# yzqin/s4g-release

Hardware: AMD Instinct MI355X
Metric: scenes/sec (25.6k-pt clouds) end-to-end grasp inference (higher is better)
Workload: dtype f32 (f16x2 split)

## Files before the change

### s4g_release_amd/csrc/mlp_gemm.hip

```cpp
#include <stdlib.h>

#include "mlp_common.h"

#include <type_traits>

#ifndef S4G_CHAIN_ABLATE
#define S4G_CHAIN_ABLATE 0
#endif

namespace s4g {


constexpr int GM_BM = 128;
constexpr int GM_BN = 128;
constexpr int GM_BK = 32;
constexpr int GM_LDS = 36;
constexpr int GM_THREADS = 256;

enum { LOAD_PLAIN = 0, LOAD_GATHER = 1, LOAD_INTERP = 2, LOAD_GATHER_MLP1 = 3, LOAD_GATHER_ADD = 4,
       LOAD_INTERP_ADD = 5, LOAD_CHANNEL_FIRST = 6,
       LOAD_REL_MLP1 = 64,
       LOAD_ADD_MFMA0 = 65 };
enum { EPI_STORE = 0, EPI_MAX = 1, EPI_CHANNEL_FIRST = 2, EPI_MAX_CF = 3 };

// ... 871 lines not shown
    for (int rb = 0; rb < 2; ++rb)
#pragma unroll
      for (int r = 0; r < 16; ++r) {
        const float v = acc[rb][cb][r] * sc;
        acc[rb][cb][r] = v;
        mx = fmaxf(mx, v);
        mn = fminf(mn, v);
      }
    const float hi = mx + bias, lo = mn + bias;
    tmax = fmaxf(tmax, p.relu ? hi : fmaxf(fabsf(hi), fabsf(lo)));
  }
  if (PL == 2 && po.out_amax) {
    const uint32_t wm = wave_max_u32(__float_as_uint(fmaxf(tmax, 0.f)));
    if (lane == 0) amax_publish(po.out_amax, wm, blockIdx.x * 4 + wave, p0, p_hi, p.rps);
  }
  if constexpr (EPI == EPI_MAX_CF)
    max_cf_epilogue<NCB>(po, acc, bg, p0, n0, wr, wc, li, lh, smemf);
  else
    gemm_epilogue<EPI, NCB>(po, acc, bg, g, p0, n0, wave, wr, wc, li, lh, smemf);
}

template <int LOADER, int EPI, int NCB, int PL>
static int launch_gemm_f16x2_cfg(GemmParams p, int groups, hipStream_t st) {
  constexpr int BN = 64 * NCB;
  p.ntiles = (p.Cout + BN - 1) / BN;
  size_t lds = sizeof(uint16_t) * PL * (GM_BM + BN) * GH_STR;
  const size_t epi = sizeof(float) * 4 * 32 * (32 * NCB + 4);
  if (lds < epi) lds = epi;
  static LdsAttrCache lds_cache;
  if (int rc = allow_dynamic_lds(reinterpret_cast<const void*>(&mlp_gemm_f16x2_kernel<LOADER, EPI, NCB, PL>), lds, lds_cache)) return rc;
  const dim3 grid((unsigned)(p.mtiles * p.ntiles), (unsigned)groups);
  hipLaunchKernelGGL((mlp_gemm_f16x2_kernel<LOADER, EPI, NCB, PL>), grid, dim3(256), lds, st, p);
  S4G_LAUNCH_CHECK();
  return S4G_OK;
}

__device__ __forceinline__ void chain_keep_alive(const f32x16& v) { asm volatile("" ::"v"(v)); }

#ifdef S4G_CHAIN_STAMPS
__device__ unsigned long long g_chain_stamps[512 * 16];
#define S4G_STAMP(i)                                                                       \
  do {                                                                                     \
    const unsigned sb_ = gridDim.x >= 1024 ? blockIdx.x - gridDim.x / 2 : blockIdx.x;    \
    if (threadIdx.x == 0 && sb_ < 512u && blockIdx.y == 0)                                 \
      g_chain_stamps[sb_ * 16 + (i)] = __builtin_amdgcn_s_memtime();                      \
  } while (0)
#else
#define S4G_STAMP(i)
#endif
constexpr int GF_RING_F16X2 = 2;
#ifndef S4G_CHAIN_RING1
#define S4G_CHAIN_RING1 2
#endif
#ifndef S4G_CHAIN_BF16_NRB
#define S4G_CHAIN_BF16_NRB 4
#endif

template <int LOADER, int EPI2, int RW, int KC, int PL>
__global__ __launch_bounds__(RW == 8 ? 512 : 256, (PL == 1 && RW != 8 && S4G_CHAIN_BF16_NRB == 2) ? 3 : 2) void mlp_chain_kernel(const GemmParams p) {
  constexpr int GF_RING = PL == 2 ? GF_RING_F16X2 : S4G_CHAIN_RING1;
  constexpr int NRB = PL == 1 ? S4G_CHAIN_BF16_NRB : 2, WROWS = 32 * NRB;
  constexpr int CW = RW == 8 ? 8 : 4 / RW, RWN = RW == 8 ? 1 : RW;
  constexpr int BM = WROWS * RWN, K = 64 * CW, NW = RWN * CW;
  constexpr int RS = 8 * NW, RPT = BM / RS;
  constexpr int astr = K + 8, aplane = BM * astr, KS = K >> 4;
  extern __shared__ __attribute__((aligned(16))) float smemf[];
  uint16_t* Ah = reinterpret_cast<uint16_t*>(smemf);
  float* scr = reinterpret_cast<float*>(Ah + PL * aplane);
  const int g = blockIdx.y;

  const int t = threadIdx.x;
  const int lane = t & 63;
  const int wave = t >> 6;

  constexpr bool ADD0 = LOADER == LOAD_ADD_MFMA0;
  constexpr bool ADD_BOUNDS = LOADER == LOAD_GATHER_ADD || LOADER == LOAD_INTERP_ADD || ADD0;
  constexpr bool MFMA0 = LOADER == LOAD_REL_MLP1;
  static_assert(!(MFMA0 || ADD0) || (PL == 2 && KC == 1), "phase 0 on the matrix cores: f16x2, one panel");
  static_assert(!ADD0 || EPI2 == EPI_MAX, "a wave's 64 rows are one centroid's neighbours");
  constexpr bool SEGMAX = (LOADER == LOAD_GATHER_MLP1 || MFMA0) && EPI2 == EPI_MAX;
  const int tile = blockIdx.x;
  const int p0 = tile * BM;
  bool seg_scene = false;
  if constexpr (SEGMAX) {
    if (p.seg_rows) {
      const int sc = p0 / p.rps;
      const int nrows = p.seg_rows[sc];
      if (p0 - sc * p.rps >= nrows) return;
      seg_scene = nrows < p.rps;
    }
  }
  const int p_hi = min(p0 + BM, p.P) - 1;
  const int am_s0 = p.rps > 0 ? p0 / p.rps : 0, am_s1 = p.rps > 0 ? p_hi / p.rps : 0;
  float am_v1 = 0.f, am_v2 = 0.f;
  if (PL == 2 && p.a_amax) am_v1 = p.a_amax[(size_t)am_s0 * 64 + lane];
  if (PL == 2 && p.a_amax2) am_v2 = p.a_amax2[(size_t)am_s0 * 64 + lane];

  const int wr = wave / CW, wc = wave % CW;
  const int li = lane & 31, lh = lane >> 5;
  const int wc_u = __builtin_amdgcn_readfirstlane(wc);
  const uint32_t wf_lane = (uint32_t)lane * 16u;
  constexpr size_t cb_stride = (size_t)KS * PL * 1024;
  constexpr size_t strip_stride = (size_t)CW * 2 * cb_stride;
  constexpr int kchunks = KC;
  const size_t cbs1 = (size_t)kchunks * cb_stride;
  const WRef w1 = wref(p.Wfrag + (size_t)g * p.Cout * p.Kpad16 * PL, (size_t)(wc_u * 2) * cbs1);
  const bool tri = p.Wfrag3 != nullptr;
  const WRef wmid = wref(p.Wfrag2 + (size_t)g * p.Cout2 * K * PL, (size_t)(wc_u * 2) * cb_stride);
  const int CoutF = tri ? p.Cout3 : p.Cout2;
  const float* __restrict__ scF = PL == 2 ? (tri ? p.w_inv_scale3 : p.w_inv_scale2) + (size_t)g * CoutF : nullptr;
  const float* __restrict__ bgF = (tri ? p.bias3 : p.bias2) + (size_t)g * CoutF;
  const WRef w2 = tri ? wref(p.Wfrag3 + (size_t)g * CoutF * K * PL, (size_t)(wc_u * 2) * cb_stride) : wmid;
  const int nstrip2 = (CoutF + 64 * CW - 1) / (64 * CW);
  const bool active0 = wc_u * 64 < CoutF;

  uint4 ring[GF_RING][2][PL];
#pragma unroll
  for (int d = 0; d < GF_RING; ++d)
#pragma unroll
    for (int cb = 0; cb < 2; ++cb)
#pragma unroll
      for (int pl = 0; pl < PL; ++pl)
        ring[d][cb][pl] = wref_load(w1, wf_lane + pl * 1024, (uint32_t)(cb * cbs1 + (size_t)d * PL * 1024));

  S4G_STAMP(0);
  ALoader<LOADER, RPT, RS> ld;
  float4 rv0[NRB];
  float4 wv0 = f4zero();
  constexpr int NKT0 = ADD0 ? K / 32 : 1, RPT0 = ADD0 ? RPT : 1;
  float4 fa[NKT0][RPT0];
  constexpr int fstr = K + 4;
  if constexpr (ADD0) {
    const int rows_left = p.P - p0;
    const __amdgpu_buffer_rsrc_t ridx = __builtin_amdgcn_make_buffer_rsrc(
        const_cast<int*>(p.gidx + p0), 0, (rows_left < BM ? rows_left : BM) * 4, 0x00020000);
    const __amdgpu_buffer_rsrc_t rxyz = __builtin_amdgcn_make_buffer_rsrc(
        const_cast<float*>(p.xyz), 0, p.nscenes * 3 * p.N * 4, 0x00020000);
    const __amdgpu_buffer_rsrc_t rfeat = __builtin_amdgcn_make_buffer_rsrc(
        const_cast<float*>(p.feat), 0, p.nscenes * p.N * p.Cf * 4, 0x00020000);
    constexpr uint32_t OOB = 0x80000000u;
    int jr[NRB], jg[RPT];
#pragma unroll
    for (int rb = 0; rb < NRB; ++rb)
      jr[rb] = __builtin_amdgcn_raw_buffer_load_b32(ridx, (wr * WROWS + rb * 32 + li) * 4, 0, 0);
#pragma unroll
    for (int s = 0; s < RPT; ++s) jg[s] = __builtin_amdgcn_raw_buffer_load_b32(ridx, ((t >> 3) + RS * s) * 4, 0, 0);
    {
      int bw, mw;
      gather_row_bm(p.M, p.K, p0, __builtin_amdgcn_readfirstlane(wr * WROWS), bw, mw);
      bw = __builtin_amdgcn_readfirstlane(bw);
      mw = __builtin_amdgcn_readfirstlane(mw);
      const bool okw = p0 + wr * WROWS < p.P;
      float cx = 0.f, cy = 0.f, cz = 0.f;
      if (okw) {
        const float* c = p.ctr + (size_t)bw * 3 * p.M + mw;
        cx = c[0];
        cy = c[p.M];
        cz = c[2 * p.M];
      }
      const uint32_t xb = okw ? (uint32_t)(bw * 3 * p.N) * 4u : OOB;
#pragma unroll
      for (int rb = 0; rb < NRB; ++rb) {
        const uint32_t vo = xb + (uint32_t)jr[rb] * 4u;
        const float x = __builtin_bit_cast(float, __builtin_amdgcn_raw_buffer_load_b32(rxyz, vo, 0, 0));
        const float y = __builtin_bit_cast(float, __builtin_amdgcn_raw_buffer_load_b32(rxyz, vo + (uint32_t)p.N * 4u, 0, 0));
        const float z = __builtin_bit_cast(float, __builtin_amdgcn_raw_buffer_load_b32(rxyz, vo + (uint32_t)p.N * 8u, 0, 0));
        rv0[rb] = make_float4(__fsub_rn(x, cx), __fsub_rn(y, cy), __fsub_rn(z, cz), 0.f);
      }
    }
    uint32_t rowoff[RPT];
#pragma unroll
    for (int s = 0; s < RPT; ++s) {
      const int c64 = (RS * s) / 64 * 64;
      int bc, mc;
      gather_row_bm(p.M, p.K, p0, c64, bc, mc);
      bc = __builtin_amdgcn_readfirstlane(bc);
      rowoff[s] = p0 + c64 < p.P ? (uint32_t)((bc * p.N + jg[s]) * p.Cf + (t & 7) * 4) * 4u : OOB;
    }
    if (p.Cin >= K) {
#pragma unroll
      for (int kt = 0; kt < NKT0; ++kt)
#pragma unroll
        for (int s = 0; s < RPT; ++s)
// ... 309 lines not shown
          tmax = fmaxf(fmaxf(tmax, fabsf(x[2])), fabsf(x[3]));
        }
      }
    }
  if constexpr (LOADER == LOAD_PLAIN && EPI2 == EPI_STORE) {
    if (!p.Wfrag2) {
      const bool second = p.split_n > 0 && g * p.c_gcol >= p.split_n;
      float* __restrict__ obase = second ? p.out2 - p.split_n : p.out + p.c_coff;
      const int old = second ? p.ldc2 : p.ldc;
      uint32_t* __restrict__ oamax = second ? p.out_amax2 : p.out_amax;
#pragma unroll
      for (int nb = 0; nb < 2; ++nb)
#pragma unroll
        for (int j = 0; j < 4; ++j) {
          const int nn = wc * 64 + nb * 32 + 8 * j + 4 * lh;
#pragma unroll
          for (int pb = 0; pb < NRB; ++pb) {
            const int row = p0 + wr * WROWS + pb * 32 + li;
            if (row < p.P)
              *reinterpret_cast<float4*>(obase + (size_t)row * old + g * p.c_gcol + nn) =
                  make_float4(acc[nb][pb][4 * j], acc[nb][pb][4 * j + 1], acc[nb][pb][4 * j + 2], acc[nb][pb][4 * j + 3]);
          }
        }
      if (PL == 2 && oamax) {
        const uint32_t wm = wave_max_u32(__float_as_uint(tmax));
        if (lane == 0) amax_publish(oamax, wm, (tile * 4 + wave) * 5 + g, p0, p_hi, p.rps);
      }
      return;
    }
  }
  float sh = 1.f;
  if constexpr (PL == 2) {
    const uint32_t wm = wave_max_u32(__float_as_uint(tmax));
    if (lane == 0) scr[NW * 128 + wave] = __uint_as_float(wm);
  }
  S4G_STAMP(5 + 4 * ph);
  __syncthreads();
  S4G_STAMP(6 + 4 * ph);
  if constexpr (PL == 2) {
    float hmax = scr[NW * 128];
#pragma unroll
    for (int w = 1; w < NW; ++w) hmax = fmaxf(hmax, scr[NW * 128 + w]);
    uint32_t exh = __float_as_uint(hmax) >> 23;
    exh = exh < 15u ? 15u : (exh > 240u ? 240u : exh);
    exh = __builtin_amdgcn_readfirstlane(exh);
    sh = __uint_as_float((268u - exh) << 23);
    inv_sh = __uint_as_float((exh - 14u) << 23);
  }
#pragma unroll
  for (int nb = 0; nb < 2; ++nb)
#pragma unroll
    for (int j = 0; j < 4; ++j)
#pragma unroll
      for (int pb = 0; pb < NRB; ++pb) {
        uint16_t* dst = Ah + (wr * WROWS + pb * 32 + li) * astr + wc * 64 + nb * 32 + 8 * j + 4 * lh;
        if constexpr (PL == 2) {
          const float4 v = make_float4(acc[nb][pb][4 * j], acc[nb][pb][4 * j + 1], acc[nb][pb][4 * j + 2],
                                       acc[nb][pb][4 * j + 3]);
          uint2 h, l;
          split2_h<false>(v, sh, h, l);
          *reinterpret_cast<uint2*>(dst) = h;
          *reinterpret_cast<uint2*>(dst + aplane) = l;
        } else {
          *reinterpret_cast<uint2*>(dst) = make_uint2(cvt_pk_bf16(acc[nb][pb][4 * j], acc[nb][pb][4 * j + 1]),
                                                      cvt_pk_bf16(acc[nb][pb][4 * j + 2], acc[nb][pb][4 * j + 3]));
        }
      }
  S4G_STAMP(7 + 4 * ph);
  __syncthreads();
  }
  inv_in = inv_sh;
  wcur = wmid;
  scp = PL == 2 ? p.w_inv_scale2 + (size_t)g * p.Cout2 : nullptr;
  bp = p.bias2 + (size_t)g * p.Cout2;
  relu_ph = p.relu2;
  }

  GemmParams q = p;
  q.Cout = CoutF;
  q.relu = tri ? p.relu3 : p.relu2;
  prime_a();
  WRef wstrip = w2;
  const float* __restrict__ bg2 = bgF;
  int sidv[NRB / 2][8] = {};
  if constexpr (SEGMAX) {
    if (seg_scene) {
#pragma unroll
      for (int c = 0; c < NRB / 2; ++c) {
        const int4* sp = reinterpret_cast<const int4*>(p.seg4 + ((p0 + wr * WROWS + c * 64 + lh * 32) >> 2));
        const int4 s0 = sp[0], s1 = sp[1];
        sidv[c][0] = s0.x; sidv[c][1] = s0.y; sidv[c][2] = s0.z; sidv[c][3] = s0.w;
        sidv[c][4] = s1.x; sidv[c][5] = s1.y; sidv[c][6] = s1.z; sidv[c][7] = s1.w;
      }
    }
  }
  for (int strip = 0; strip < nstrip2; ++strip, wstrip = wstrip + strip_stride) {
    if ((strip * CW + wc_u) * 64 >= CoutF) break;
    const int n = (strip * CW + wc) * 64 + lane;
    const float e_sc = PL == 2 ? inv_sh * scF[n] : 1.f;
    const float e_bias = bg2[n];
    const WRef wnext = ((strip + 1) * CW + wc_u) * 64 < CoutF ? wstrip + strip_stride : wstrip;
    S4G_STAMP(12 + 2 * (strip & 1));
    S4G_F2_STRIP(EPI2 == EPI_STORE, true, wstrip, cb_stride, wnext, cb_stride)
    S4G_STAMP(13 + 2 * (strip & 1));
    if (S4G_CHAIN_ABLATE & 8) {
      chain_keep_alive(acc[0][0]); chain_keep_alive(acc[0][1]); chain_keep_alive(acc[1][0]); chain_keep_alive(acc[1][1]);
      continue;
    }
    const int n0 = (strip * CW + wc) * 64;
    float omax = 0.f;
    if constexpr (EPI2 == EPI_STORE) {
      epi_s[lane] = e_sc;
      epi_s[64 + lane] = e_bias;
#pragma unroll
      for (int nb = 0; nb < 2; ++nb)
#pragma unroll
        for (int j = 0; j < 4; ++j) {
          const int nn = n0 + nb * 32 + 8 * j + 4 * lh;
          const float4 sc4 = *reinterpret_cast<const float4*>(epi_s + nb * 32 + 8 * j + 4 * lh);
          const float4 b4 = *reinterpret_cast<const float4*>(epi_s + 64 + nb * 32 + 8 * j + 4 * lh);
          const float scv[4] = {sc4.x, sc4.y, sc4.z, sc4.w};
          const float bv[4] = {b4.x, b4.y, b4.z, b4.w};
#pragma unroll
          for (int pb = 0; pb < NRB; ++pb) {
            float v[4];
#pragma unroll
            for (int e = 0; e < 4; ++e) {
              float x = __fmaf_rn(acc[nb][pb][4 * j + e], scv[e], bv[e]);
              if (q.relu) x = fmaxf(x, 0.f);
              v[e] = x;
              omax = fmaxf(omax, fabsf(x));
            }
            const int row = p0 + wr * WROWS + pb * 32 + li;
            if (row < p.P)
              *reinterpret_cast<float4*>(p.out + (size_t)row * p.ldc + p.c_coff + g * p.c_gcol + nn) =
                  make_float4(v[0], v[1], v[2], v[3]);
          }
        }
      if (p.out_amax) {
        const uint32_t wm = wave_max_u32(__float_as_uint(omax));
        if (lane == 0) amax_publish(p.out_amax, wm, tile * 4 + wave + strip, p0, p_hi, p.rps);
      }
    } else if (SEGMAX && seg_scene) {
      uint32_t* __restrict__ outu = reinterpret_cast<uint32_t*>(p.out);
#pragma unroll
      for (int cb = 0; cb < 2; ++cb) {
        const float sc = __shfl(e_sc, cb * 32 + li);
        const float bias = __shfl(e_bias, cb * 32 + li);
        const int nn = n0 + cb * 32 + li;
#pragma unroll
        for (int c = 0; c < NRB / 2; ++c) {
        float v[8];
#pragma unroll
        for (int qd = 0; qd < 4; ++qd) {
          const float o0 = fmaxf(fmaxf(acc[cb][2 * c][4 * qd], acc[cb][2 * c][4 * qd + 1]),
                                 fmaxf(acc[cb][2 * c][4 * qd + 2], acc[cb][2 * c][4 * qd + 3]));
          const float o1 = fmaxf(fmaxf(acc[cb][2 * c + 1][4 * qd], acc[cb][2 * c + 1][4 * qd + 1]),
                                 fmaxf(acc[cb][2 * c + 1][4 * qd + 2], acc[cb][2 * c + 1][4 * qd + 3]));
          const auto r = __builtin_amdgcn_permlane32_swap(__float_as_uint(o0), __float_as_uint(o1), false, false);
          v[2 * qd] = __uint_as_float(r[0]);
          v[2 * qd + 1] = __uint_as_float(r[1]);
        }
        auto emit = [&](int seg, float m) {
          if (seg < 0) return;
          const float x = fmaxf(m * sc + bias, 0.f);
          omax = fmaxf(omax, x);
          if (nn < CoutF) atomicMax(outu + (size_t)seg * p.ldc + p.c_coff + nn, __float_as_uint(x));
        };
        int cur = sidv[c][0];
        float m = v[0];
#pragma unroll
        for (int i = 1; i < 8; ++i) {
          const bool chg = sidv[c][i] != cur;
          if (chg) emit(cur, m);
          m = chg ? v[i] : fmaxf(m, v[i]);
          cur = sidv[c][i];
        }
        emit(cur, m);
        }
      }
      if (PL == 2 && p.out_amax) {
        const uint32_t wm = wave_max_u32(__float_as_uint(omax));
        if (lane == 0) amax_publish(p.out_amax, wm, tile * 4 + wave + strip, p0, p_hi, p.rps);
      }
    } else if (q.relu && p.K == 64) {
#pragma unroll
      for (int cb = 0; cb < 2; ++cb) {
        const float sc = __shfl(e_sc, cb * 32 + li);
        const float bias = __shfl(e_bias, cb * 32 + li);
        const int nn = n0 + cb * 32 + li;
#pragma unroll
        for (int c = 0; c < NRB / 2; ++c) {
          float m = acc[cb][2 * c][0];
#pragma unroll
          for (int rb = 2 * c; rb < 2 * c + 2; ++rb)
#pragma unroll
            for (int r = 0; r < 16; ++r) m = fmaxf(m, acc[cb][rb][r]);
          m = fmaxf(m, __shfl_xor(m, 32));
          const float v = fmaxf(m * sc + bias, 0.f);
          omax = fmaxf(omax, v);
          const int row0 = p0 + wr * WROWS + c * 64;
          if (nn < CoutF && lh == 0 && row0 < p.P) p.out[(size_t)(row0 >> 6) * p.ldc + p.c_coff + nn] = v;
        }
      }
      if (PL == 2 && p.out_amax) {
        const uint32_t wm = wave_max_u32(__float_as_uint(omax));
        if (lane == 0) amax_publish(p.out_amax, wm, tile * 4 + wave + strip, p0, p_hi, p.rps);
      }
    } else if constexpr (NRB == 2) {
      f32x16 acct[2][2];
#pragma unroll
      for (int cb = 0; cb < 2; ++cb) {
        const float sc = __shfl(e_sc, cb * 32 + li);
        const float bias = __shfl(e_bias, cb * 32 + li);
        float mx = -__builtin_inff(), mn = __builtin_inff();
#pragma unroll
        for (int rb = 0; rb < 2; ++rb)
#pragma unroll
          for (int r = 0; r < 16; ++r) {
            const float v = acc[cb][rb][r] * sc;
            acct[rb][cb][r] = v;
            mx = fmaxf(mx, v);
            mn = fminf(mn, v);
          }
        const float hi = mx + bias, lo = mn + bias;
        omax = fmaxf(omax, q.relu ? hi : fmaxf(fabsf(hi), fabsf(lo)));
      }
      if (p.out_amax) {
        const uint32_t wm = wave_max_u32(__float_as_uint(fmaxf(omax, 0.f)));
        if (lane == 0) amax_publish(p.out_amax, wm, tile * 4 + wave + strip, p0, p_hi, p.rps);
      }
      gemm_epilogue<EPI_MAX, 2>(q, acct, bg2, g, p0, n0, wave, wr, 0, li, lh, smemf);
    }
  }
  S4G_STAMP(11);
#undef S4G_F2_STRIP
#undef S4G_F2_TERM
}

template <int LOADER, int EPI2, int RW, int KC, int PL>
static int launch_mlp_chain(const GemmParams& p, int groups, hipStream_t st) {
  constexpr int CW = RW == 8 ? 8 : 4 / RW, RWN = RW == 8 ? 1 : RW;
  constexpr int NRB = PL == 1 ? S4G_CHAIN_BF16_NRB : 2;
  constexpr int BM = 32 * NRB * RWN, K = 64 * CW, NW = RWN * CW;
  constexpr size_t lds = sizeof(uint16_t) * PL * BM * (size_t)(K + 8) + sizeof(float) * (NW * 128 + 16);
  static_assert(lds <= (RW == 8 ? 160 : 80) * 1024, "two workgroups per CU (one for the 8-wave form)");
  static LdsAttrCache lds_cache;
  if (int rc = allow_dynamic_lds(reinterpret_cast<const void*>(&mlp_chain_kernel<LOADER, EPI2, RW, KC, PL>), lds, lds_cache)) return rc;
  const dim3 grid((unsigned)((p.P + BM - 1) / BM), (unsigned)groups);
  hipLaunchKernelGGL((mlp_chain_kernel<LOADER, EPI2, RW, KC, PL>), grid, dim3(64 * NW), lds, st, p);
  S4G_LAUNCH_CHECK();
  return S4G_OK;
}

template <int LOADER, int EPI, int PL = 2>
static int launch_gemm_f16x2(const GemmParams& p, int groups, hipStream_t st) {
  constexpr int force = 0;
  const int64_t wide_wgs = (int64_t)((p.P + GM_BM - 1) / GM_BM) * ((p.Cout + 255) / 256) * groups;
  const bool wide = force ? force == 4
                          : p.Cout > 256 && wide_wgs >= 512 &&
                                (LOADER == LOAD_PLAIN || LOADER == LOAD_GATHER_MLP1 || LOADER == LOAD_GATHER_ADD);
  if (wide) return launch_gemm_f16x2_cfg<LOADER, EPI, 4, PL>(p, groups, st);
  return launch_gemm_f16x2_cfg<LOADER, EPI, 2, PL>(p, groups, st);
}

template <int LOADER, int EPI, int NS, int WAVES>
static int launch_gemm_bf16x3_cfg(const GemmParams& p, int groups, hipStream_t st) {
  constexpr int BK = 32 * NS;
  size_t lds = sizeof(float) * GM_BM * (BK + 4) + sizeof(uint16_t) * 3 * GM_BN * (BK + 8);
  const size_t epi = sizeof(float) * 4 * 32 * 68;
  if (lds < epi) lds = epi;
  static LdsAttrCache lds_cache;
  if (int rc = allow_dynamic_lds(reinterpret_cast<const void*>(&mlp_gemm_bf16x3_kernel<LOADER, EPI, NS, WAVES>), lds, lds_cache)) return rc;
  const dim3 grid((unsigned)(p.mtiles * p.ntiles), (unsigned)groups);
  hipLaunchKernelGGL((mlp_gemm_bf16x3_kernel<LOADER, EPI, NS, WAVES>), grid, dim3(64 * WAVES), lds,
                     st, p);
  S4G_LAUNCH_CHECK();
  return S4G_OK;
}

template <int LOADER, int EPI>
static int launch_gemm_bf16x3(const GemmParams& p, int groups, hipStream_t st) {
  return launch_gemm_bf16x3_cfg<LOADER, EPI, 1, 4>(p, groups, st);
}

template <int LOADER, int EPI>
static int launch_gemm(const GemmParams& p, int groups, hipStream_t st) {
  const size_t lds = sizeof(float) * 2 * (GM_BM + GM_BN) * GM_LDS;
  static LdsAttrCache lds_cache;
  if (int rc = allow_dynamic_lds(reinterpret_cast<const void*>(&mlp_gemm_kernel<LOADER, EPI>), lds, lds_cache)) return rc;
  const dim3 grid((unsigned)(p.mtiles * p.ntiles), (unsigned)groups);
  hipLaunchKernelGGL((mlp_gemm_kernel<LOADER, EPI>), grid, dim3(GM_THREADS), lds, st, p);
  S4G_LAUNCH_CHECK();
  return S4G_OK;
}

}

#define S4G_FUSED2_LIST(X)                                                                       \
  X(LOAD_GATHER_MLP1, EPI_MAX, 2, 1)                                                             \
  X(LOAD_GATHER_MLP1, EPI_MAX, 1, 1)                                                             \
  X(LOAD_GATHER_ADD, EPI_MAX, 2, 1)                                                              \
  X(LOAD_GATHER_ADD, EPI_MAX, 1, 1)                                                              \
  X(LOAD_GATHER_ADD, EPI_MAX, 8, 1)       \
  X(LOAD_PLAIN, EPI_MAX, 2, 1)                                                                   \
  X(LOAD_PLAIN, EPI_MAX, 1, 1)                                                                   \
  X(LOAD_PLAIN, EPI_MAX, 8, 1)                                                                   \
  X(LOAD_PLAIN, EPI_STORE, 2, 1)                                                                 \
  X(LOAD_PLAIN, EPI_STORE, 1, 1)                                                                 \
  X(LOAD_PLAIN, EPI_STORE, 1, 2)            \
  X(LOAD_PLAIN, EPI_STORE, 1, 4)         \
  X(LOAD_PLAIN, EPI_STORE, 8, 1)                                                                 \
  X(LOAD_INTERP_ADD, EPI_STORE, 2, 1)                                                            \
  X(LOAD_INTERP_ADD, EPI_STORE, 1, 1)                                                            \
  X(LOAD_INTERP_ADD, EPI_STORE, 8, 1)

// ... 14 lines not shown
#undef S4G_FUSED2_Q
  return 0;
}

extern "C" int s4g_mlp_gemm_f32(const s4g_gemm_desc_t* d, s4g_stream_t stream) {
  using namespace s4g;
  if (!d || d->P < 0 || d->Cout <= 0 || d->groups <= 0 || !d->bias) return S4G_EINVAL;
  const bool split = d->precision == S4G_GEMM_BF16X3 || d->precision == S4G_GEMM_BF16;
  const bool h2 = d->precision == S4G_GEMM_F16X2;
  if (h2) {
    if (!d->W_f16x2 || !d->w_inv_scale || d->Kpad16 <= 0 || (d->Kpad16 & 15) ||
        !(d->a_amax_floor >= 0.f) || (!d->a_amax && !d->a_amax2 && !(d->a_amax_floor > 0.f)))
      return S4G_EINVAL;
  } else if (split) {
    if (!d->W_bf16x3 || d->Kpad16 <= 0 || (d->Kpad16 & 15)) return S4G_EINVAL;
  } else if (d->precision == S4G_GEMM_FP32) {
    if (!d->W || d->Kpad <= 0 || (d->Kpad & 7)) return S4G_EINVAL;
  } else {
    return S4G_EINVAL;
  }
  if (d->P == 0) return S4G_OK;
  GemmParams p;
  p.P = d->P; p.Cin = d->Cin; p.Kpad = d->Kpad; p.Cout = d->Cout; p.relu = d->relu;
  p.W = d->W; p.bias = d->bias;
  p.A = d->A; p.lda = d->lda; p.a_coff = d->a_coff; p.a_gcol = d->a_gcol; p.aL = d->a_L;
  p.gidx = d->gidx; p.feat = d->feat; p.xyz = d->xyz; p.ctr = d->ctr;
  p.Cf = d->Cf; p.N = d->N; p.M = d->M; p.K = d->K;
  p.nscenes = d->M > 0 && d->K > 0 ? (int)((d->P + (int64_t)d->M * d->K - 1) / ((int64_t)d->M * d->K)) : 0;
  p.mlp1 = (const float4*)d->mlp1_w;
  p.rel4 = (const float4*)d->rel_xyz4;
  p.seg4 = d->seg4;
  p.seg_rows = d->seg_rows;
  p.out2 = d->out2;
  p.ldc2 = d->ldc2;
  p.split_n = d->out2 ? d->split_n : 0;
  p.out_amax2 = (uint32_t*)d->out_amax2;
  p.nidx = d->nidx; p.nw = d->nw; p.sparse = d->sparse; p.dense = d->dense;
  p.C2 = d->C2; p.C1 = d->C1; p.N2 = d->N2; p.N1 = d->N1;
  p.out = d->out; p.ldc = d->ldc; p.c_coff = d->c_coff; p.c_gcol = d->c_gcol;
  p.w_gstride = d->w_gstride; p.b_gstride = d->b_gstride;
  for (int i = 0; i < 4; ++i) p.cf_ptr[i] = d->cf_ptr[i];
  for (int i = 0; i < 5; ++i) p.cf_start[i] = d->cf_start[i];
  p.cf_sigmoid_from = d->cf_sigmoid_from; p.cf_N = d->cf_N;
  p.W3 = (const uint16_t*)d->W_bf16x3;
  p.Kpad16 = d->Kpad16;
  p.bf16_single = d->precision == S4G_GEMM_BF16 ? 1 : 0;
  p.w3_plane = (size_t)d->groups * (size_t)d->Cout * (size_t)d->Kpad16;
  p.Wh2 = (const uint16_t*)d->W_f16x2;
  p.w_inv_scale = d->w_inv_scale;
  p.a_amax = d->a_amax; p.a_amax2 = d->a_amax2; p.a_amax_floor = d->a_amax_floor;
  p.out_amax = (uint32_t*)d->out_amax;
  p.rps = d->rows_per_scene > 0 ? d->rows_per_scene : 0;
  p.Wfrag = (const uint16_t*)d->W_f16x2_frag;
  p.lbias = d->loader_bias;
  p.Wfrag2 = (const uint16_t*)d->W2_f16x2_frag;
  p.w_inv_scale2 = d->w2_inv_scale;
  p.bias2 = d->bias2;
  p.Cout2 = d->Cout2;
  p.relu2 = d->relu2;
  p.Wfrag3 = (const uint16_t*)d->W3_f16x2_frag;
  p.w_inv_scale3 = d->w3_inv_scale;
  p.bias3 = d->bias3;
  p.Cout3 = d->Cout3;
  p.relu3 = d->relu3;
  p.mtiles = (d->P + GM_BM - 1) / GM_BM;
  p.ntiles = (d->Cout + GM_BN - 1) / GM_BN;
  hipStream_t st = (hipStream_t)stream;

  if (d->loader == S4G_GEMM_LOAD_PLAIN) {
    if (!d->A || (d->lda & 3) || (d->a_coff & 3) || (d->a_gcol & 3) || (d->Cin & 3)) return S4G_EINVAL;
  } else if (d->loader == S4G_GEMM_LOAD_GATHER) {
    if (!d->gidx || !d->xyz || !d->ctr || (d->Cf & 3) || (d->Cf > 0 && !d->feat) ||
        d->K <= 0 || d->M <= 0 || d->N <= 0 || d->groups != 1)
      return S4G_EINVAL;
  } else if (d->loader == S4G_GEMM_LOAD_GATHER_MLP1) {
    if ((!d->rel_xyz4 && (!d->gidx || !d->xyz || !d->ctr)) || ((uintptr_t)d->rel_xyz4 & 15) ||
        !d->mlp1_w || (d->Cin & 3) || d->K <= 0 || d->M <= 0 || d->N <= 0 || d->groups != 1 ||
        ((uintptr_t)d->mlp1_w & 15))
      return S4G_EINVAL;
    if ((d->seg4 != nullptr) != (d->seg_rows != nullptr)) return S4G_EINVAL;
    if (d->seg4 && (!d->rel_xyz4 || !d->W2_f16x2_frag || d->epilogue != S4G_GEMM_EPI_MAX || d->K != 64 ||
                    d->rows_per_scene <= 0 || (d->rows_per_scene & 255) || !d->relu2 || d->W3_f16x2_frag))
      return S4G_EINVAL;
  } else if (d->loader == S4G_GEMM_LOAD_GATHER_ADD) {
    if (!d->gidx || !d->xyz || !d->ctr || !d->mlp1_w || !d->feat || (d->Cin & 3) || d->Cf != d->Cin ||
        d->K <= 0 || d->M <= 0 || d->N <= 0 || d->groups != 1 || ((uintptr_t)d->mlp1_w & 15) ||
        ((uintptr_t)d->feat & 15))
      return S4G_EINVAL;
  } else if (d->loader == S4G_GEMM_LOAD_INTERP_ADD) {
    if (!d->nidx || !d->nw || !d->sparse || !d->loader_bias || (d->Cin & 3) || d->C2 != d->Cin ||
        d->N1 <= 0 || d->N2 <= 0 || d->groups != 1 ||
        (((uintptr_t)d->sparse | (uintptr_t)d->dense | (uintptr_t)d->loader_bias) & 15))
      return S4G_EINVAL;
  } else if (d->loader == S4G_GEMM_LOAD_INTERP) {
    if (!d->nidx || !d->nw || !d->sparse || (d->C2 & 3) || (d->C1 & 3) ||
        (d->C1 > 0 && !d->dense) || d->N1 <= 0 || d->N2 <= 0 || d->groups != 1)
      return S4G_EINVAL;
  } else if (d->loader == S4G_GEMM_LOAD_CHANNEL_FIRST) {
    if (!d->A || d->Cin < 1 || d->a_L <= 0 || d->P % d->a_L || d->groups != 1 ||
        d->Cin > (h2 ? d->Kpad16 : d->Kpad))
      return S4G_EINVAL;
  } else {
    return S4G_EINVAL;
  }
  if (d->loader != S4G_GEMM_LOAD_GATHER_MLP1 && (d->seg4 || d->seg_rows)) return S4G_EINVAL;
  if (d->out2) {
    const bool bf1_ = d->precision == S4G_GEMM_BF16;
    if (!(h2 || bf1_) || d->loader != S4G_GEMM_LOAD_PLAIN || d->epilogue != S4G_GEMM_EPI_STORE || d->W2_f16x2_frag ||
        d->groups != 1 || d->split_n <= 0 || (d->split_n & 255) || d->split_n >= d->Cout || (d->Cout & 255) ||
        (d->ldc2 & 3) || ((uintptr_t)d->out2 & 15) || d->c_coff != 0 || (d->ldc & 3) || ((uintptr_t)d->out & 15))
      return S4G_EINVAL;
  }
  if (d->epilogue == S4G_GEMM_EPI_MAX) {
    if (!(d->K == 16 || d->K == 32 || d->K == 64) || d->groups != 1 || !d->out) return S4G_EINVAL;
  } else if (d->epilogue == S4G_GEMM_EPI_STORE) {
    if (!d->out) return S4G_EINVAL;
  } else if (d->epilogue == S4G_GEMM_EPI_CHANNEL_FIRST) {
    if (d->cf_N <= 0 || d->groups != 1) return S4G_EINVAL;
  } else if (d->epilogue == S4G_GEMM_EPI_MAX_CHANNEL_FIRST) {
    if (d->relu != 1 || d->K < 1 || d->M < 1 || d->P % ((int64_t)d->M * d->K) || d->groups != 1 || !d->out ||
        d->W2_f16x2_frag || d->out2)
      return S4G_EINVAL;
  } else {
    return S4G_EINVAL;
  }

  if (d->W2_f16x2_frag) {
    const bool c128 = d->Cout == 128 && d->Kpad16 == 128,
               c256 = d->Cout == 256 && (d->Kpad16 == 256 || d->Kpad16 == 512 || d->Kpad16 == 1024),
               c512 = d->Cout == 512 && d->Kpad16 == 512;
    const bool store = d->epilogue == S4G_GEMM_EPI_STORE;
    const bool bf1 = d->precision == S4G_GEMM_BF16;
    if ((!h2 && !bf1) || (!store && (d->epilogue != S4G_GEMM_EPI_MAX || d->K != 64 || (d->P & 63))) ||
        (!c128 && !c256 && !c512) || d->Cout2 <= 0 || (d->Cout2 & 63) || (!store && d->groups != 1) || !d->W_f16x2_frag ||
        (d->W3_f16x2_frag && (d->Cout2 != d->Cout || d->Cout3 <= 0 || (d->Cout3 & 63) ||
                              (h2 && !d->w3_inv_scale) || !d->bias3)) ||
        (h2 && !d->w2_inv_scale) || !d->bias2 ||
        (store && (((d->ldc | d->c_coff | d->c_gcol) & 3) || ((uintptr_t)d->out & 15))))
      return S4G_EINVAL;
    if (bf1 && !store && !(d->W3_f16x2_frag ? d->relu3 : d->relu2)) return S4G_EUNSUPPORTED;
    if (h2 && d->loader == S4G_GEMM_LOAD_GATHER_MLP1 && d->rel_xyz4 && d->epilogue == S4G_GEMM_EPI_MAX &&
        d->Kpad16 == d->Cout && d->Cin <= d->Cout && (c128 || c256)) {
      const char* m0 = s4g::knob("S4G_MLP1_MFMA");
      if (!(m0 && m0[0] == '0'))
        return c128 ? launch_mlp_chain<LOAD_REL_MLP1, EPI_MAX, 2, 1, 2>(p, d->groups, st)
                    : launch_mlp_chain<LOAD_REL_MLP1, EPI_MAX, 1, 1, 2>(p, d->groups, st);
    }
    if (h2 && d->loader == S4G_GEMM_LOAD_GATHER_ADD && d->epilogue == S4G_GEMM_EPI_MAX && d->Kpad16 == d->Cout &&
        (int64_t)p.nscenes * d->N * d->Cf * 4 < (1ll << 31) && (int64_t)p.nscenes * d->N * 12 < (1ll << 31))
      return c128   ? launch_mlp_chain<LOAD_ADD_MFMA0, EPI_MAX, 2, 1, 2>(p, d->groups, st)
             : c256 ? launch_mlp_chain<LOAD_ADD_MFMA0, EPI_MAX, 1, 1, 2>(p, d->groups, st)
                    : launch_mlp_chain<LOAD_ADD_MFMA0, EPI_MAX, 8, 1, 2>(p, d->groups, st);
#define S4G_FUSED2_CASE(L, E, R, KCH)                                                        \
  if (d->loader == L && (int)d->epilogue == (int)E && (c128 ? 2 : (c256 ? 1 : 8)) == R &&     \
      d->Kpad16 / d->Cout == KCH)                                                             \
    return bf1 ? launch_mlp_chain<L, E, R, KCH, 1>(p, d->groups, st)                 \
               : launch_mlp_chain<L, E, R, KCH, 2>(p, d->groups, st);
    S4G_FUSED2_LIST(S4G_FUSED2_CASE)
#undef S4G_FUSED2_CASE
    return S4G_EUNSUPPORTED;
  }
  {
    const char* sc_env = s4g::knob("S4G_GEMM_SINGLE_CHAIN");
    const bool single_chain = !(sc_env && sc_env[0] == '0');
    const bool bf1 = d->precision == S4G_GEMM_BF16;
    const int kc = d->Kpad16 / 256;
// ... 74 lines not shown
```

Before: 1992.

## Streamline fused MLP chain max epilogues: precomputed segment offsets, single amax publish

Reworks the epilogue of the fused MLP chain kernel. Segment ids are loaded once per tile and redistributed by shuffle, with the atomic target byte offsets and segment-boundary limits precomputed outside the strip loop, so the segmented max needs fewer branches and less address arithmetic. The per-column scale and bias loads now avoid shuffles, the K=64 max path reduces halves with permlane32_swap and has all lanes store, and the amax reduction and publish happen once per wave after all strips instead of once per strip. In exchange, register pressure rises from the precomputed per-segment arrays, and a host check rejects outputs whose offsets would not fit in 32 bits.

```diff
diff --git a/s4g_release_amd/csrc/mlp_gemm.hip b/s4g_release_amd/csrc/mlp_gemm.hip
--- a/s4g_release_amd/csrc/mlp_gemm.hip
+++ b/s4g_release_amd/csrc/mlp_gemm.hip
@@ -977,12 +977,14 @@
   const int tile = blockIdx.x;
   const int p0 = tile * BM;
   bool seg_scene = false;
+  int seg_tile = -1;
   if constexpr (SEGMAX) {
     if (p.seg_rows) {
       const int sc = p0 / p.rps;
       const int nrows = p.seg_rows[sc];
       if (p0 - sc * p.rps >= nrows) return;
       seg_scene = nrows < p.rps;
+      if (lane < BM / 4) seg_tile = p.seg4[(p0 >> 2) + lane];
     }
   }
   const int p_hi = min(p0 + BM, p.P) - 1;
@@ -993,7 +995,7 @@
 
   const int wr = wave / CW, wc = wave % CW;
   const int li = lane & 31, lh = lane >> 5;
-  const int wc_u = __builtin_amdgcn_readfirstlane(wc);
+  const int wc_u = __builtin_amdgcn_readfirstlane(wc), wr_u = __builtin_amdgcn_readfirstlane(wr);
   const uint32_t wf_lane = (uint32_t)lane * 16u;
   constexpr size_t cb_stride = (size_t)KS * PL * 1024;
   constexpr size_t strip_stride = (size_t)CW * 2 * cb_stride;
@@ -1469,23 +1471,47 @@
   prime_a();
   WRef wstrip = w2;
   const float* __restrict__ bg2 = bgF;
-  int sidv[NRB / 2][8] = {};
+  constexpr uint32_t SEG_NONE = 0xFFFFFFFFu;
+  uint32_t seg_off[NRB / 2][8] = {};
+  float seg_lim[NRB / 2][8] = {};
+  uint32_t seg_any[NRB / 2] = {};
   if constexpr (SEGMAX) {
     if (seg_scene) {
 #pragma unroll
       for (int c = 0; c < NRB / 2; ++c) {
-        const int4* sp = reinterpret_cast<const int4*>(p.seg4 + ((p0 + wr * WROWS + c * 64 + lh * 32) >> 2));
-        const int4 s0 = sp[0], s1 = sp[1];
-        sidv[c][0] = s0.x; sidv[c][1] = s0.y; sidv[c][2] = s0.z; sidv[c][3] = s0.w;
-        sidv[c][4] = s1.x; sidv[c][5] = s1.y; sidv[c][6] = s1.z; sidv[c][7] = s1.w;
-      }
-    }
-  }
+        int sid[8];
+#pragma unroll
+        for (int i = 0; i < 8; ++i) sid[i] = __shfl(seg_tile, wr * (WROWS / 4) + c * 16 + lh * 8 + i);
+        uint32_t mine = 0u;
+#pragma unroll
+        for (int i = 0; i < 8; ++i) {
+          const bool ends = i == 7 || sid[i + 1] != sid[i];
+          const bool merges = ends && sid[i] >= 0;
+          seg_off[c][i] = merges ? ((uint32_t)sid[i] * (uint32_t)p.ldc + (uint32_t)p.c_coff + (uint32_t)li) * 4u : SEG_NONE;
+          seg_lim[c][i] = (i > 0 && sid[i] != sid[i - 1]) ? -__builtin_inff() : __builtin_inff();
+          mine |= merges ? 1u << i : 0u;
+        }
+        seg_any[c] = __builtin_amdgcn_readlane(mine, 0) | __builtin_amdgcn_readlane(mine, 32);
+      }
+    }
+  }
+  float omax = 0.f;
   for (int strip = 0; strip < nstrip2; ++strip, wstrip = wstrip + strip_stride) {
     if ((strip * CW + wc_u) * 64 >= CoutF) break;
-    const int n = (strip * CW + wc) * 64 + lane;
-    const float e_sc = PL == 2 ? inv_sh * scF[n] : 1.f;
-    const float e_bias = bg2[n];
+    const int n0u = (strip * CW + wc_u) * 64;
+    constexpr bool PER_BLOCK = EPI2 != EPI_STORE && SEGMAX;
+    [[maybe_unused]] float e_sc = 1.f, e_bias = 0.f, sc2[2] = {1.f, 1.f}, bias2[2] = {0.f, 0.f};
+    if constexpr (!PER_BLOCK) {
+      const int n = (PL == 2 ? n0u : (strip * CW + wc) * 64) + lane;
+      e_sc = PL == 2 ? inv_sh * scF[n] : 1.f;
+      e_bias = bg2[n];
+    } else {
+#pragma unroll
+      for (int cb = 0; cb < 2; ++cb) {
+        sc2[cb] = PL == 2 ? inv_sh * scF[n0u + cb * 32 + li] : 1.f;
+        bias2[cb] = bg2[n0u + cb * 32 + li];
+      }
+    }
     const WRef wnext = ((strip + 1) * CW + wc_u) * 64 < CoutF ? wstrip + strip_stride : wstrip;
     S4G_STAMP(12 + 2 * (strip & 1));
     S4G_F2_STRIP(EPI2 == EPI_STORE, true, wstrip, cb_stride, wnext, cb_stride)
@@ -1495,7 +1521,6 @@
       continue;
     }
     const int n0 = (strip * CW + wc) * 64;
-    float omax = 0.f;
     if constexpr (EPI2 == EPI_STORE) {
       epi_s[lane] = e_sc;
       epi_s[64 + lane] = e_bias;
@@ -1524,82 +1549,78 @@
                   make_float4(v[0], v[1], v[2], v[3]);
           }
         }
-      if (p.out_amax) {
-        const uint32_t wm = wave_max_u32(__float_as_uint(omax));
-        if (lane == 0) amax_publish(p.out_amax, wm, tile * 4 + wave + strip, p0, p_hi, p.rps);
-      }
     } else if (SEGMAX && seg_scene) {
-      uint32_t* __restrict__ outu = reinterpret_cast<uint32_t*>(p.out);
+      char* __restrict__ outb = reinterpret_cast<char*>(p.out + n0u);
 #pragma unroll
       for (int cb = 0; cb < 2; ++cb) {
-        const float sc = __shfl(e_sc, cb * 32 + li);
-        const float bias = __shfl(e_bias, cb * 32 + li);
-        const int nn = n0 + cb * 32 + li;
+        const float sc = sc2[cb], bias = bias2[cb];
+        const bool nn_ok = n0u + cb * 32 + li < CoutF;
 #pragma unroll
         for (int c = 0; c < NRB / 2; ++c) {
         float v[8];
 #pragma unroll
         for (int qd = 0; qd < 4; ++qd) {
-          const float o0 = fmaxf(fmaxf(acc[cb][2 * c][4 * qd], acc[cb][2 * c][4 * qd + 1]),
-                                 fmaxf(acc[cb][2 * c][4 * qd + 2], acc[cb][2 * c][4 * qd + 3]));
-          const float o1 = fmaxf(fmaxf(acc[cb][2 * c + 1][4 * qd], acc[cb][2 * c + 1][4 * qd + 1]),
-                                 fmaxf(acc[cb][2 * c + 1][4 * qd + 2], acc[cb][2 * c + 1][4 * qd + 3]));
+          const float o0 = fmaxf(fmaxf(fmaxf(acc[cb][2 * c][4 * qd], acc[cb][2 * c][4 * qd + 1]), acc[cb][2 * c][4 * qd + 2]),
+                                 acc[cb][2 * c][4 * qd + 3]);
+          const float o1 = fmaxf(fmaxf(fmaxf(acc[cb][2 * c + 1][4 * qd], acc[cb][2 * c + 1][4 * qd + 1]),
+                                       acc[cb][2 * c + 1][4 * qd + 2]), acc[cb][2 * c + 1][4 * qd + 3]);
           const auto r = __builtin_amdgcn_permlane32_swap(__float_as_uint(o0), __float_as_uint(o1), false, false);
           v[2 * qd] = __uint_as_float(r[0]);
           v[2 * qd + 1] = __uint_as_float(r[1]);
         }
-        auto emit = [&](int seg, float m) {
-          if (seg < 0) return;
-          const float x = fmaxf(m * sc + bias, 0.f);
-          omax = fmaxf(omax, x);
-          if (nn < CoutF) atomicMax(outu + (size_t)seg * p.ldc + p.c_coff + nn, __float_as_uint(x));
-        };
-        int cur = sidv[c][0];
         float m = v[0];
 #pragma unroll
-        for (int i = 1; i < 8; ++i) {
-          const bool chg = sidv[c][i] != cur;
-          if (chg) emit(cur, m);
-          m = chg ? v[i] : fmaxf(m, v[i]);
-          cur = sidv[c][i];
-        }
-        emit(cur, m);
-        }
-      }
-      if (PL == 2 && p.out_amax) {
-        const uint32_t wm = wave_max_u32(__float_as_uint(omax));
-        if (lane == 0) amax_publish(p.out_amax, wm, tile * 4 + wave + strip, p0, p_hi, p.rps);
+        for (int i = 0; i < 8; ++i) {
+          if (i > 0) m = fmaxf(fminf(m, seg_lim[c][i]), v[i]);
+          if (seg_any[c] & (1u << i)) {
+            if (seg_off[c][i] != SEG_NONE) {
+              const float x = fmaxf(m * sc + bias, 0.f);
+              omax = fmaxf(omax, x);
+              uint32_t off = seg_off[c][i];
+              asm volatile("" : "+v"(off));
+              if (nn_ok) atomicMax(reinterpret_cast<uint32_t*>(outb + cb * 128 + off), __float_as_uint(x));
+            }
+          }
+        }
+        }
       }
     } else if (q.relu && p.K == 64) {
-#pragma unroll
-      for (int cb = 0; cb < 2; ++cb) {
-        const float sc = __shfl(e_sc, cb * 32 + li);
-        const float bias = __shfl(e_bias, cb * 32 + li);
-        const int nn = n0 + cb * 32 + li;
-#pragma unroll
-        for (int c = 0; c < NRB / 2; ++c) {
-          float m = acc[cb][2 * c][0];
-#pragma unroll
-          for (int rb = 2 * c; rb < 2 * c + 2; ++rb)
-#pragma unroll
-            for (int r = 0; r < 16; ++r) m = fmaxf(m, acc[cb][rb][r]);
-          m = fmaxf(m, __shfl_xor(m, 32));
-          const float v = fmaxf(m * sc + bias, 0.f);
-          omax = fmaxf(omax, v);
+      const float sc = PER_BLOCK ? (lh ? sc2[1] : sc2[0]) : e_sc, bias = PER_BLOCK ? (lh ? bias2[1] : bias2[0]) : e_bias;
+      const int nn = n0 + lane;
+#pragma unroll
+      for (int c = 0; c < NRB / 2; ++c) {
+        float mb[2];
+#pragma unroll
+        for (int cb = 0; cb < 2; ++cb) {
+          float mr[2];
+#pragma unroll
+          for (int rb = 0; rb < 2; ++rb) {
+            float m = acc[cb][2 * c + rb][0];
+#pragma unroll
+            for (int r = 1; r < 15; r += 2) m = fmaxf(fmaxf(m, acc[cb][2 * c + rb][r]), acc[cb][2 * c + rb][r + 1]);
+            mr[rb] = m;
+          }
+          mb[cb] = fmaxf(fmaxf(fmaxf(mr[0], acc[cb][2 * c][15]), acc[cb][2 * c + 1][15]), mr[1]);
+        }
+        const auto hs = __builtin_amdgcn_permlane32_swap(__float_as_uint(mb[0]), __float_as_uint(mb[1]), false, false);
+        const float m = fmaxf(__uint_as_float(hs[0]), __uint_as_float(hs[1]));
+        const float v = fmaxf(m * sc + bias, 0.f);
+        omax = fmaxf(omax, v);
+        if constexpr (PL == 2) {
+          const int row0 = p0 + wr_u * WROWS + c * 64;
+          float* __restrict__ orow = p.out + (size_t)(row0 >> 6) * p.ldc + p.c_coff + n0u;
+          if (nn < CoutF && row0 < p.P) orow[lane] = v;
+        } else {
           const int row0 = p0 + wr * WROWS + c * 64;
-          if (nn < CoutF && lh == 0 && row0 < p.P) p.out[(size_t)(row0 >> 6) * p.ldc + p.c_coff + nn] = v;
-        }
-      }
-      if (PL == 2 && p.out_amax) {
-        const uint32_t wm = wave_max_u32(__float_as_uint(omax));
-        if (lane == 0) amax_publish(p.out_amax, wm, tile * 4 + wave + strip, p0, p_hi, p.rps);
+          if (nn < CoutF && row0 < p.P) p.out[(size_t)(row0 >> 6) * p.ldc + p.c_coff + nn] = v;
+        }
       }
     } else if constexpr (NRB == 2) {
       f32x16 acct[2][2];
 #pragma unroll
       for (int cb = 0; cb < 2; ++cb) {
-        const float sc = __shfl(e_sc, cb * 32 + li);
-        const float bias = __shfl(e_bias, cb * 32 + li);
+        const float sc = PER_BLOCK ? sc2[cb] : __shfl(e_sc, cb * 32 + li);
+        const float bias = PER_BLOCK ? bias2[cb] : __shfl(e_bias, cb * 32 + li);
         float mx = -__builtin_inff(), mn = __builtin_inff();
 #pragma unroll
         for (int rb = 0; rb < 2; ++rb)
@@ -1613,12 +1634,12 @@
         const float hi = mx + bias, lo = mn + bias;
         omax = fmaxf(omax, q.relu ? hi : fmaxf(fabsf(hi), fabsf(lo)));
       }
-      if (p.out_amax) {
-        const uint32_t wm = wave_max_u32(__float_as_uint(fmaxf(omax, 0.f)));
-        if (lane == 0) amax_publish(p.out_amax, wm, tile * 4 + wave + strip, p0, p_hi, p.rps);
-      }
       gemm_epilogue<EPI_MAX, 2>(q, acct, bg2, g, p0, n0, wave, wr, 0, li, lh, smemf);
     }
+  }
+  if (active0 && p.out_amax && (PL == 2 || EPI2 == EPI_STORE)) {
+    const uint32_t wm = wave_max_u32(__float_as_uint(omax));
+    if (lane == 0) amax_publish(p.out_amax, wm, tile * 4 + wave, p0, p_hi, p.rps);
   }
   S4G_STAMP(11);
 #undef S4G_F2_STRIP
@@ -1799,6 +1820,7 @@
     if (d->seg4 && (!d->rel_xyz4 || !d->W2_f16x2_frag || d->epilogue != S4G_GEMM_EPI_MAX || d->K != 64 ||
                     d->rows_per_scene <= 0 || (d->rows_per_scene & 255) || !d->relu2 || d->W3_f16x2_frag))
       return S4G_EINVAL;
+    if (d->seg4 && ((int64_t)(d->P >> 6) * d->ldc + d->c_coff) * 4 + 256 > (int64_t)0xFFFFFFFF) return S4G_EUNSUPPORTED;
   } else if (d->loader == S4G_GEMM_LOAD_GATHER_ADD) {
     if (!d->gidx || !d->xyz || !d->ctr || !d->mlp1_w || !d->feat || (d->Cin & 3) || d->Cf != d->Cin ||
         d->K <= 0 || d->M <= 0 || d->N <= 0 || d->groups != 1 || ((uintptr_t)d->mlp1_w & 15) ||
```

Result: no change. 2012, median of 6 (+1.0%).
